# andabi/parallel-wavenet-vocoder

Measured on AMD Instinct MI355X. Metric: audio samples/sec, 4-flow IAF generation, higher is better.
Workload: dtype f32 via 3-term split-fp16 MFMA (fp32 accumulate, fp32 storage)

## Files before the change

parallel-wavenet-vocoder_amd/csrc/pwv_f16x3.h:

```cpp
#pragma once

#include "pwv_layer_common.h"

namespace pwv {

typedef float f32x2 __attribute__((ext_vector_type(2)));

template <int OFF, int N>
__device__ __forceinline__ void split8(const float (&x)[N], f16x8& hi, f16x8& lo) {
#pragma unroll
    for (int q = 0; q < 8; q += 2) {
        const f32x2 v = {x[OFF + q], x[OFF + q + 1]};
        const f16x2 h = __builtin_convertvector(v, f16x2);
        f32x2 r;
        asm("v_fma_mix_f32 %0, %1, -1.0, %2 op_sel:[0,0,0] op_sel_hi:[1,0,0]" : "=v"(r[0]) : "v"(h), "v"(v[0]));
        asm("v_fma_mix_f32 %0, %1, -1.0, %2 op_sel:[1,0,0] op_sel_hi:[1,0,0]" : "=v"(r[1]) : "v"(h), "v"(v[1]));
        const f16x2 l = __builtin_convertvector(r, f16x2);
        hi[q] = h[0];
        hi[q + 1] = h[1];
        lo[q] = l[0];
        lo[q + 1] = l[1];
    }
}

template <int NS, int NITTOT>
__device__ __forceinline__ f16x8 frag16(const f16x8* A, int comp, int it, int s, int lane) {
    return A[((comp * NITTOT + it) * NS + s) * 64 + lane];
}

template <int NS, int NIT, int IT0, int ITSTEP, int NITTOT, int NACC, typename BH, typename BL, typename EF, typename TF>
__device__ __forceinline__ void gemm16(const f16x8* A, int lane, f32x16 (&acc)[NACC], f16x8 (&ah)[4], f16x8 (&al)[4],
                                       BH&& bh, BL&& bl, EF&& extra, TF&& tail) {
#pragma unroll
    for (int s = 0; s < NS; ++s) {
        f16x8 nh[4] = {ah[0], ah[1], ah[2], ah[3]};
        f16x8 nl[4] = {al[0], al[1], al[2], al[3]};
        if (s + 1 < NS) {
#pragma unroll
            for (int i = 0; i < NIT; ++i) {
                nh[i] = frag16<NS, NITTOT>(A, 0, IT0 + i * ITSTEP, s + 1, lane);
                nl[i] = frag16<NS, NITTOT>(A, 1, IT0 + i * ITSTEP, s + 1, lane);
            }
        } else {
            tail(nh, nl);
        }
        __builtin_amdgcn_sched_barrier(0);
// ... 53 lines not shown
            ah[i] = nh[i];
            al[i] = nl[i];
        }
    }
}

template <int NS, int S, int NIT, int IT0, int ITSTEP, int NITTOT>
__device__ __forceinline__ void frags_at(const f16x8* A, int lane, f16x8 (&h)[4], f16x8 (&l)[4]) {
#pragma unroll
    for (int i = 0; i < NIT; ++i) {
        h[i] = frag16<NS, NITTOT>(A, 0, IT0 + i * ITSTEP, S, lane);
        l[i] = frag16<NS, NITTOT>(A, 1, IT0 + i * ITSTEP, S, lane);
    }
}

template <int NS, int NIT, int IT0, int ITSTEP, int NITTOT>
__device__ __forceinline__ void first_frags(const f16x8* A, int lane, f16x8 (&h)[4], f16x8 (&l)[4]) {
#pragma unroll
    for (int i = 0; i < NIT; ++i) {
        h[i] = frag16<NS, NITTOT>(A, 0, IT0 + i * ITSTEP, 0, lane);
        l[i] = frag16<NS, NITTOT>(A, 1, IT0 + i * ITSTEP, 0, lane);
    }
}

}
```

parallel-wavenet-vocoder_amd/csrc/pwv_head_f32.inc:

```
            PWV_HEAD_FENCE();
            f32x16 accs[4];
#pragma unroll
            for (int it = 0; it < 4; ++it)
#pragma unroll
                for (int q = 0; q < 4; ++q) {
                    const f32x4 v = *reinterpret_cast<const f32x4*>(hb + kHBS + h * 64 + it * 16 + q * 4);
#pragma unroll
                    for (int e = 0; e < 4; ++e) accs[it][q * 4 + e] = v[e];
                }
#pragma unroll
            for (int r = 0; r < 16; ++r) o[16 + r] = gate_act(acc[1][r], acc[3][r]);
            gemm_groups<8, 4, 0, 1>(lds, kHS, lane, accs, a, [&](int ks) -> float { return o[ks]; }, no_extra,
                                    [&](f32x4(&n)[4]) {
#pragma unroll
                                        for (int i = 0; i < 4; ++i) n[i] = frag(lds, kH1, i, 16, 0, lane);
                                    });
            PWV_HEAD_FENCE();
#pragma unroll
            for (int it = 0; it < 4; ++it)
#pragma unroll
                for (int q = 0; q < 4; ++q) {
                    const f32x4 v = *reinterpret_cast<const f32x4*>(hb + kHB1 + h * 64 + it * 16 + q * 4);
#pragma unroll
                    for (int e = 0; e < 4; ++e) acc1[it][q * 4 + e] = v[e];
                }
            gemm_groups<16, 4, 0, 1>(
                lds, kH1, lane, acc1, a, [&](int ks) -> float { return fmaxf(accs[ks >> 4][ks & 15], 0.f); }, no_extra,
                [](f32x4(&)[4]) {});
```

parallel-wavenet-vocoder_amd/csrc/pwv_layer_common.h:

```cpp
#pragma once

#include "pwv_common.h"

namespace pwv {

constexpr int kA1 = 0;
constexpr int kA1Size = 4 * 16 * 64 * 4;
constexpr int kA2 = kA1 + kA1Size;
constexpr int kA2Size = 2 * 8 * 64 * 4;
constexpr int kBD = kA2 + kA2Size;
constexpr int kBDSize = 64;
constexpr int kLayerBase = kBD + kBDSize;
constexpr int kASSize = 4 * 8 * 64 * 4;
constexpr int kBSSize = 128;
constexpr int kCondC = 80;
constexpr int kACSize = 4 * (kCondC / 8) * 64 * 4;

constexpr int layer_floats(bool skip, bool cond) {
    return kLayerBase + (skip ? kASSize + kBSSize : 0) + (cond ? kACSize : 0);
}

constexpr int kHAS = 0;
constexpr int kHBS = kHAS + kASSize;
constexpr int kHA1 = kHBS + kBSSize;
// ... 207 lines not shown
template <int NCH>
__device__ __forceinline__ void load_contig(const float* __restrict__ p, float (&dst)[4 * NCH]) {
#pragma unroll
    for (int g = 0; g < NCH; ++g) {
        const f32x4 v = *reinterpret_cast<const f32x4*>(p + 4 * g);
#pragma unroll
        for (int e = 0; e < 4; ++e) dst[4 * g + e] = v[e];
    }
}


__device__ __forceinline__ f32x4 frag(const float* lds, int base, int it, int ngroups, int g, int lane) {
    return *reinterpret_cast<const f32x4*>(&lds[base + ((it * ngroups + g) * 64 + lane) * 4]);
}

template <int NG, int NIT, int IT0, int ITSTEP, int NACC, typename BF, typename EF, typename TF>
__device__ __forceinline__ void gemm_groups(const float* lds, int base, int lane, f32x16 (&acc)[NACC], f32x4 (&a)[4],
                                            BF&& bval, EF&& extra, TF&& tail) {
#pragma unroll
    for (int g = 0; g < NG; ++g) {
        f32x4 n[4] = {a[0], a[1], a[2], a[3]};
        if (g + 1 < NG) {
#pragma unroll
            for (int i = 0; i < NIT; ++i) n[i] = frag(lds, base, IT0 + i * ITSTEP, NG, g + 1, lane);
        } else {
            tail(n);
        }
        __builtin_amdgcn_sched_barrier(0);
#pragma unroll
        for (int e = 0; e < 4; ++e) {
            const float b = bval(g * 4 + e);
#pragma unroll
// ... 28 lines not shown
```

parallel-wavenet-vocoder_amd/csrc/pwv_layer_f32_body.inc:

```
    static_assert(!FOLD || FIRST, "FOLD: layer 0 of a scalar-input net only");
    static_assert(!STREAM || (!SKIP && !COND && FOLD == FIRST && GATED == HEAD), "STREAM: folded layer 0, plain residual layer, last layer + head");
    static_assert(!HEAD || (GATED && !SKIP && !COND && !FIRST), "HEAD: plain last layer only");
    static_assert(!FIRST || !SKIP, "FIRST: no skip accumulation");
    constexpr int WAVES = 8;
    constexpr int kLds = HEAD ? kA1Size + kASSize + kHA1Size : layer_floats(SKIP, COND);
    constexpr int kCF = kLds + 4;
    constexpr int kHS = kA1Size;
    constexpr int kH1 = kA1Size + kASSize;
    __shared__ __attribute__((aligned(16))) float lds[kLds + (HEAD ? 0 : 4) + (FIRST ? 128 : 0)];

    const int tid = threadIdx.x;
    const int lane = tid & 63;
    const int wave = __builtin_amdgcn_readfirstlane(tid >> 6);
    const int h = lane >> 5;
    const int net = blockIdx.x % p.G;
    const int wg = blockIdx.x / p.G;
    const int nwg = gridDim.x / p.G;
    int* unit_counter = reinterpret_cast<int*>(&lds[HEAD ? 0 : kLds]);

    if constexpr (HEAD) {
        fill_lds_dma<kA1Size / 4, WAVES>(lds, p.packed[net] + kA1, wave, lane);
        fill_lds_dma<kASSize / 4, WAVES>(lds + kHS, p.packed_head[net] + kHAS, wave, lane);
        fill_lds_dma<kHA1Size / 4, WAVES>(lds + kH1, p.packed_head[net] + kHA1, wave, lane);
    } else {
// ... 151 lines not shown
                    n[1] = frag(lds, kA2, 1, 8, 0, lane);
                } else if constexpr (SKIP) {
#pragma unroll
                    for (int i = 0; i < 4; ++i) n[i] = frag(lds, kAS, i, 8, 0, lane);
                } else if constexpr (HEAD) {
#pragma unroll
                    for (int i = 0; i < 4; ++i) n[i] = frag(lds, kHS, i, 8, 0, lane);
                }
            });
        }

        const int ooff = units_off(cur.row, h, 64, u_begin);
        if constexpr (GATED && HEAD) {
            const float* hb = p.packed_head[net];
            f32x16 acc1[4];
#define PWV_HEAD_FENCE() do {} while (0)
#include "pwv_head_f32.inc"
#undef PWV_HEAD_FENCE
            const int Q = p.head_q;
            const int hq = h * Q;
#define PWV_HEAD_STORE(q, part) if (cur.valid && h == 0) p.head_out[net][(size_t)cur.row * Q + (q)] = (part)
#include "pwv_head_pp2.inc"
#undef PWV_HEAD_STORE
        } else if constexpr (GATED) {
            if constexpr (SKIP) load_skip_row<SKIP, COND>(p, net, lane, cur, skip_load);
#pragma unroll
            for (int r = 0; r < 16; ++r) o[16 + r] = gate_act(acc[1][r], acc[3][r]);
            if (cur.valid) {
#pragma unroll
                for (int g = 0; g < 8; ++g) {
// ... 79 lines not shown
```

parallel-wavenet-vocoder_amd/csrc/pwv_persist_fold0.inc:

```
    if (p.x_first && p.fold0[net]) {
        const float* Af = lds;
        const f16x8* A2 = reinterpret_cast<const f16x8*>(lds + kA1Size);
        (void)Af;
        (void)A2;
        const float* bias = lds + kBiasF + h * 32;
        const char* F0 = reinterpret_cast<const char*>(p.fold0[net]);
        const float* lastfrag = packed_n + kSlot + lane * 4;
        const int d = dil_of(0);
        const int dn = dil_next(0);
        typedef const __attribute__((address_space(3))) f32x4* lds_f4_t;
        const lds_f4_t cfb = (lds_f4_t)(lds + kCfF + 4 * h);
        f16x8 fh[4], fl[4];
        f32x4 ff[4];
#pragma unroll
        for (int it = 0; it < 4; ++it) {
            if constexpr (F32) {
                ff[it] = *reinterpret_cast<const f32x4*>(F0 + it * 1024 + lane * 16);
            } else {
                fh[it] = *reinterpret_cast<const f16x8*>(F0 + it * 1024 + lane * 16);
                fl[it] = *reinterpret_cast<const f16x8*>(F0 + (4 + it) * 1024 + lane * 16);
            }
        }
        const f32x4 lf32 = *reinterpret_cast<const f32x4*>(lastfrag);
        while (u >= 0 && j == 0) {
// ... 34 lines not shown
                int prow = 0;
                if (p.cond_hop > 0) prow = p_base(nn) + fast_div(t + p.cond_offset, p.hop_magic, p.hop_shift);
                const float* pr = proj_n + (size_t)prow * p.proj_row_stride + h * 64;
#pragma unroll
                for (int it = 0; it < 4; ++it)
#pragma unroll
                    for (int q = 0; q < 4; ++q) {
                        const f32x4 v = *reinterpret_cast<const f32x4*>(pr + it * 16 + q * 4);
#pragma unroll
                        for (int e = 0; e < 4; ++e) acc[it][q * 4 + e] = v[e];
                    }
            }
            int j2 = 0;
            const int u2 = next_task(0, u, j2);
            asm volatile("s_waitcnt vmcnt(0)" ::: "memory");
            publish();
            if (u2 >= 0 && !stat) claim_v = claim();
            if (p.range_flag && !(fabsf(x0) <= p.x_limit)) __hip_atomic_store(p.range_flag, 1, __ATOMIC_RELAXED, __HIP_MEMORY_SCOPE_SYSTEM);
            if constexpr (F32) {
                const float b0 = h ? xd0 : xd1, b1 = h ? x0 : x1v;
#pragma unroll
                for (int it = 0; it < 4; ++it) acc[it] = __builtin_amdgcn_mfma_f32_32x32x2f32(ff[it][0], b0, acc[it], 0, 0, 0);
#pragma unroll
                for (int it = 0; it < 4; ++it) acc[it] = __builtin_amdgcn_mfma_f32_32x32x2f32(ff[it][1], b1, acc[it], 0, 0, 0);
            } else {
                f16x8 b_h = {0, 0, 0, 0, 0, 0, 0, 0}, b_l = {0, 0, 0, 0, 0, 0, 0, 0};
                const float sc[4] = {xd1, xd0, x1v, x0};
#pragma unroll
                for (int q = 0; q < 4; ++q) {
                    const float v = h == 0 ? sc[q] : 0.f;
// ... 77 lines not shown
```

parallel-wavenet-vocoder_amd/csrc/pwv_persist_geometry.inc:

```
    constexpr bool SHORT = MODE == 2;
    __shared__ __attribute__((aligned(16))) float lds[kLdsFloats];
    const int tid = threadIdx.x;
    const int lane = tid & 63;
    const int wave = __builtin_amdgcn_readfirstlane(tid >> 6);
    const int h = lane >> 5;

    int net, w;
    if (p.xcd_map) {
        const int x = blockIdx.x & 7, s = blockIdx.x >> 3;
        net = s % p.G;
        w = x * (p.nwg >> 3) + s / p.G;
    } else {
        net = blockIdx.x % p.G;
        w = blockIdx.x / p.G;
    }
    const int rows = p.N * p.T;
    auto rows_of = [&](int unit, int& row, bool& valid, int& rc, int& nn, int& t) {
        if constexpr (VARLEN) unit_rows_varlen(p.unit_map, unit, lane, rows, row, valid, rc, nn, t);
        else unit_rows(unit, lane, rows, p.N, p.T, p.T_magic, p.T_shift, row, valid, rc, nn, t);
    };
    constexpr int kLaneStride = kMaxPLayers, kLaneHopMagic = kMaxPLayers + 1, kLaneHopShift = kMaxPLayers + 2, kLaneCondOffset = kMaxPLayers + 3,
                  kLaneCondFrames = kMaxPLayers + 4;
    static_assert(kMaxPLayers + 5 <= 64, "the dilations and the P row's scalars share one VGPR");
    int v_dil = p.dil[lane & (kMaxPLayers - 1)];
    if constexpr (!SHORT) {
        const int k = lane - kMaxPLayers;
        const int c = k == 0 ? p.proj_row_stride : (k == 1 ? (int)p.hop_magic : (k == 2 ? (int)p.hop_shift : (k == 3 ? p.cond_offset : p.cond_frames)));
        v_dil = k >= 0 ? c : v_dil;
    }
    auto dil_of = [&](int j) -> int { return __builtin_amdgcn_readlane(v_dil, j); };
    auto top_scalar = [&](int k) -> int { return __builtin_amdgcn_readlane(v_dil, k); };
    (void)top_scalar;
    auto p_base = [&](int nn) -> int {
        if constexpr (VARLEN) return nn;
        else if constexpr (SHORT) return nn * p.cond_frames;
        else return nn * top_scalar(kLaneCondFrames);
    };
    constexpr bool RAGGED = VARLEN && STREAM;
    auto unit_rec = [&](int unit, int& s0, int& r1) {
        typedef const __attribute__((address_space(4))) int* const_ints_t;
        const int last = (rows - 1) >> 5;
        const const_ints_t rec = (const_ints_t)(p.unit_map + (size_t)(unit < last ? unit : last) * kVarlenRec);
// ... 3 lines not shown
    auto session_end = [&](int s0, int r1, bool second) -> int {
        return second ? p.cu_rows[s0 + 2] : r1;
    };
    (void)unit_rec;
    (void)session_end;
    const int u_begin = w * p.per_wg;
    const int u_end = u_begin + p.per_wg < p.units ? u_begin + p.per_wg : p.units;
    const int n = u_end - u_begin;
    if (n <= 0) return;
    const int L = p.n_layers;
    constexpr bool stat = SHORT;
    constexpr bool loader_mode = SHORT;
#ifdef PWV_PTRACE
    int pt_nev = 0;
#endif

    typedef __attribute__((address_space(3))) int* lds_ints_t;
    const lds_ints_t ctl = (lds_ints_t)(lds + kCtlF);
    typedef __attribute__((address_space(3))) volatile unsigned char* lds_bytes_t;
    const lds_bytes_t lb = (lds_bytes_t)lds;
    int* prog_n = p.prog + (size_t)net * p.nwg * kProgStride;
    int* uprog_n = p.uprog + (size_t)net * p.units * kUnitStride;
    const float* const proj_n = p.proj[net];
    const float* const packed_n = p.packed[net];
    auto dil_next = [&](int j) -> int { return j + 1 < L ? dil_of(j + 1) : (p.tail_q > 0 ? p.tail_dil : dil_of(j)); };

    for (int k = tid; k < (kLdsFloats - kCtlF); k += 512) ctl[k] = 0;
    __syncthreads();
    if (tid == 0) {
        lb[kSeenLB] = w > 0 ? 0 : 255;
        lb[kSeenRB] = w < p.last_wg ? 0 : 255;
        lb[kWreadyB] = 0;
        lb[kWreadyB + 1] = 1;
        lb[kTrueB] = 255;
    }
    auto fill_slot = [&](int slot, int layer, int first, int step) {
        const float* src = packed_n + (size_t)layer * p.packed_stride + lane * 4;
        float* dst = lds + slot * kSlot;
        if constexpr (!SHORT) {
            const __amdgpu_buffer_rsrc_t prs = __builtin_amdgcn_make_buffer_rsrc((void*)(packed_n + (size_t)layer * p.packed_stride), 0, (kSlotFull + 64) * 4, 0x00020000);
#pragma clang loop unroll(disable)
            for (int c = first; c < kSlot / 256; c += step)
                __builtin_amdgcn_raw_ptr_buffer_load_lds(prs, (lptr_t)(dst + c * 256), 16, lane * 16, c * 1024, 0, 0);
            if (first == 0 && lane < 16) __builtin_amdgcn_raw_ptr_buffer_load_lds(prs, (lptr_t)(lds + kBiasF + slot * 64), 16, lane * 16, kSlotFull * 4, 0, 0);
            return;
        }
#pragma clang loop unroll(disable)
        for (int c = first; c < kSlot / 256; c += step)
            __builtin_amdgcn_global_load_lds((gptr_t)(src + c * 256), (lptr_t)(dst + c * 256), 16, 0, 0);
        if (first == 0 && lane < 16)
            __builtin_amdgcn_global_load_lds((gptr_t)(src + kSlotFull), (lptr_t)(lds + kBiasF + slot * 64), 16, 0, 0);
    };
    if (p.x_first && tid < 128) lds[kCfF + tid] = p.cfilt[net][tid];
    fill_slot(0, 0, wave, 8);
    if (L > 1) fill_slot(1, 1, wave, 8);
    __syncthreads();
    if (wave >= 4) __builtin_amdgcn_s_setprio(1);

    const __amdgpu_buffer_rsrc_t ring_rs = [&]() {
        const unsigned long long a = (unsigned long long)p.ring[net];
        const unsigned long long span = (unsigned long long)p.ring_stride * 8ull + (unsigned long long)p.units * 8192ull;
        const unsigned lo = __builtin_amdgcn_readfirstlane((unsigned)a), hi2 = __builtin_amdgcn_readfirstlane((unsigned)(a >> 32));
        return __builtin_amdgcn_make_buffer_rsrc((void*)(((unsigned long long)hi2 << 32) | lo), 0, __builtin_amdgcn_readfirstlane((unsigned)span), 0x00020000);
    }();
    const __amdgpu_buffer_rsrc_t proj_rs = [&]() {
        const unsigned long long a = (unsigned long long)proj_n;
        const unsigned lo = __builtin_amdgcn_readfirstlane((unsigned)a), hi2 = __builtin_amdgcn_readfirstlane((unsigned)(a >> 32));
        return __builtin_amdgcn_make_buffer_rsrc((void*)(((unsigned long long)hi2 << 32) | lo), 0, 0xFFFFFFFFu, 0x00020000);
    }();
    (void)proj_rs;
    auto proj_rs_at = [&](long long floats) -> __amdgpu_buffer_rsrc_t {
// ... 153 lines not shown
```

parallel-wavenet-vocoder_amd/csrc/pwv_persist_loader.inc:

```
    if (loader_mode && wave == 7) {
        __builtin_amdgcn_s_setprio(0);
        bool gone = false;
        for (int jj = 0; jj < L && !gone; ++jj) {
            const long long t0 = __builtin_amdgcn_s_memrealtime();
            for (int k = 0;; ++k) {
                if (__builtin_amdgcn_readfirstlane(*(__attribute__((address_space(3))) volatile int*)&ctl[8 + jj]) >= n) break;
                if (__builtin_amdgcn_readfirstlane(*(__attribute__((address_space(3))) volatile int*)&ctl[1])) { gone = true; break; }
                if ((k & 63) == 63 && (__builtin_amdgcn_readfirstlane(__hip_atomic_load(p.abort, __ATOMIC_RELAXED, __HIP_MEMORY_SCOPE_AGENT)) ||
                                       __builtin_amdgcn_s_memrealtime() - t0 > kWaitTicks)) {
                    __hip_atomic_store(p.status, 7, __ATOMIC_RELAXED, __HIP_MEMORY_SCOPE_SYSTEM);
                    __hip_atomic_store(p.abort, 1, __ATOMIC_RELAXED, __HIP_MEMORY_SCOPE_AGENT);
                    *(__attribute__((address_space(3))) volatile int*)&ctl[1] = 1;
                    gone = true;
                    break;
                }
                __builtin_amdgcn_s_sleep(2);
            }
            if (gone) break;
            if (lane == 0) __hip_atomic_store(prog_n + (size_t)w * kProgStride, jj + 1, __ATOMIC_RELAXED, __HIP_MEMORY_SCOPE_AGENT);
            PT_EV(7, jj, -1);
            if (jj + 2 < L) {
                fill_slot(jj & 1, jj + 2, 0, 1);
                asm volatile("s_waitcnt vmcnt(0)" ::: "memory");
                lb[kWreadyB + (jj & 1)] = (unsigned char)(jj + 2);
            }
        }
    }
```

parallel-wavenet-vocoder_amd/csrc/pwv_persist_plan.h:

```cpp
#pragma once

#include <cstddef>

#include "pwv_hip.h"

#ifndef PWV_CHECK_ARG
#define PWV_CHECK_ARG(cond, ...)          \
    do {                                  \
        if (!(cond)) return PWV_EINVAL;   \
    } while (0)
#endif

namespace pwv {

constexpr int kLeftN = 32;
constexpr int kUnitModeMaxPerWg = 7;
constexpr int kUnitStride = 32;
constexpr int kMaxPLayers = 32;
constexpr int kProgStride = 32;
constexpr int kMaxReachWgs = 60;
constexpr int kMaxUnitsWg = 832;
constexpr int kPlanMaxQ = 4;

struct PersistPlan { int units, nwg, per_wg, last_wg, reach_wgs, xcd_map, tail_reach_wgs, unit_mode; };
// ... 28 lines not shown
    pl.unit_mode = 0;
    if (reach <= kLeftN && pl.nwg > 1 && pl.per_wg <= kUnitModeMaxPerWg) {
        pl.unit_mode = 2;
        PWV_CHECK_ARG(pl.reach_wgs <= 32, "persistent stack: unit mode polls at most 32 right neighbours (reach %d workgroups)", pl.reach_wgs);
    }
    pl.tail_reach_wgs = 0;
    if (tail_q > 0) {
        PWV_CHECK_ARG(tail_q <= kPlanMaxQ && tail_dil >= 1, "persistent stack: tail_q 1..%d, tail_dilation >= 1", kPlanMaxQ);
        PWV_CHECK_ARG(rows * tail_q * 4 < (1ll << 32), "persistent stack: tail_out beyond the 4 GB reach of a buffer descriptor");
        pl.tail_reach_wgs = ((tail_dil + 31) / 32 + pl.per_wg - 1) / pl.per_wg;
        PWV_CHECK_ARG(pl.tail_reach_wgs <= kMaxReachWgs, "persistent stack: tail dilation %d reaches over %d workgroups (max %d)", tail_dil, pl.tail_reach_wgs, kMaxReachWgs);
    }
    return PWV_OK;
}

struct PersistLayout { size_t prog_bytes, pair_off, uprog_off, total; };

inline size_t align256(size_t v) { return (v + 255) & ~(size_t)255; }

inline PersistLayout persist_layout(int G, const PersistPlan& pl) {
    PersistLayout l;
    l.prog_bytes = (size_t)G * pl.nwg * kProgStride * 4;
    l.pair_off = align256(l.prog_bytes + 256);
    l.uprog_off = l.pair_off + align256((size_t)pl.nwg * 4);
    l.total = l.uprog_off + (pl.unit_mode ? align256((size_t)G * pl.units * kUnitStride * 4) : 0);
    return l;
}

}
```

parallel-wavenet-vocoder_amd/csrc/pwv_persist_protocol.inc:

```

    int vpack = 0;
    auto layer_vectors = [&](int j) {
        const int d = dil_of(j), d2 = dil_of(j >= 2 ? j - 2 : 0);
        const int off = lane == 1 ? -((d + 31) >> 5) : (lane == 2 ? -(d >> 5) : (lane == 4 ? (d2 >> 5) : (lane == 5 ? ((d2 + 31) >> 5) : 0)));
        const int raw = j >= 1 ? j : 0, wts = j >= 2 ? j : 0, war = j >= 2 ? j - 1 : 0;
        const int need = lane < 3 ? raw : (lane == 3 ? wts : (lane < 6 ? war : 0));
        vpack = (need << 16) | (off & 0xffff);
    };
    auto dep_addr = [&](int j, int u) -> int {
        const int v = u + (int)(short)vpack;
        int a = kDoneB - u_begin + v;
        a = (v < u_begin && !SHORT) ? kSeenLB : a;
        a = v >= u_end ? kSeenRB : a;
        a = (v < 0 || v >= p.units) ? kTrueB : a;
        a = lane == 3 ? kWreadyB + (j & 1) : a;
        return lane >= 6 ? kTrueB : a;
    };
    auto eval = [&](int addr) -> unsigned { return (unsigned)__ballot((int)lb[addr] < (vpack >> 16)); };
    auto wave_min = [&](int v) -> int {
#pragma unroll
        for (int o = 32; o >= 1; o >>= 1) { const int t = __shfl_xor(v, o); v = t < v ? t : v; }
        return v;
    };
    auto poll_side = [&](int side, int need) {
// ... 20 lines not shown
            v = __hip_atomic_load(uprog_n + (size_t)(u_begin - kLeftN + addr - kLeftB) * kUnitStride, __ATOMIC_RELAXED, __HIP_MEMORY_SCOPE_AGENT);
        } else if (lo >= 32 && lo - 32 < cnt_r) {
            v = __hip_atomic_load(prog_n + (size_t)(w + 1 + lo - 32) * kProgStride, __ATOMIC_RELAXED, __HIP_MEMORY_SCOPE_AGENT);
        }
        v = v > 255 ? 255 : v;
        if (left) lb[addr] = (unsigned char)v;
        if (cnt_r > 0) {
            const bool r = lo >= 32;
            if (__ballot(r && v < jw + 1) == 0) lb[kSeenRB] = (unsigned char)(jw + 1);
            else if (__ballot(r && v < jw) == 0 && (int)lb[kSeenRB] < jw) lb[kSeenRB] = (unsigned char)jw;
        }
    };

    int prev_addr = -1, prev_j = 0;
    int dma_pending = -1;
    int left_upto = 0;
    bool dead = false;
    auto publish = [&]() {
        if (prev_addr >= 0) {
            lb[prev_addr] = (unsigned char)(prev_j + 1);
            if (SHORT && lane == 0) __hip_atomic_store(uprog_n + (size_t)(prev_addr - kDoneB + u_begin) * kUnitStride, prev_j + 1, __ATOMIC_RELAXED, __HIP_MEMORY_SCOPE_AGENT);
            prev_addr = -1;
        }
        if (dma_pending >= 0) { lb[kWreadyB + (dma_pending & 1)] = (unsigned char)dma_pending; dma_pending = -1; }
    };
    auto flush_owed = [&]() {
        asm volatile("s_waitcnt vmcnt(0)" ::: "memory");
        publish();
    };
    auto leave_layers = [&](int upto) {
        for (; left_upto < upto; ++left_upto) {
            const int jj = left_upto;
            int old = 0;
            if (lane == 0) old = __hip_atomic_fetch_add(&ctl[8 + jj], 1, __ATOMIC_RELAXED, __HIP_MEMORY_SCOPE_WORKGROUP);
            old = __builtin_amdgcn_readfirstlane(old);
            if (old == 7 && !loader_mode) {
                if (lane == 0) __hip_atomic_store(prog_n + (size_t)w * kProgStride, jj + 1, __ATOMIC_RELAXED, __HIP_MEMORY_SCOPE_AGENT);
                PT_EV(7, jj, -1);
                if (jj + 2 < L) {
                    if (dma_pending >= 0) flush_owed();
                    fill_slot(jj & 1, jj + 2, 0, 1);
                    dma_pending = jj + 2;
                }
            }
        }
    };
    auto wait_deps = [&](int j, int u, unsigned mask, int lv, int code) {
        if (!SHORT || prev_addr >= 0 || dma_pending >= 0) {
            flush_owed();
            PT_EV(mask == kWarMask ? 13 : 3, j, u);
        }
        leave_layers(j);
        if (dma_pending >= 0) flush_owed();
        if (lv != j) layer_vectors(j);
        const int addr = dep_addr(j, u);
        bool ok = false;
        const long long t0 = __builtin_amdgcn_s_memrealtime();
// ... 56 lines not shown
```

parallel-wavenet-vocoder_amd/csrc/pwv_persist_tail.inc:

```
    bool tail_done = false;
    {
        if (p.tail_q > 0) {
            tail_done = true;
            PT_EV(8, L, -1);
            __syncthreads();
            const int wg_dead = __builtin_amdgcn_readfirstlane(*(__attribute__((address_space(3))) volatile int*)&ctl[1]);
            __syncthreads();
            bool tail_ok = !wg_dead;
            if (tail_ok) {
                constexpr int kHS = kA1Size, kH1 = kA1Size + kASSize;
                fill_lds_dma<kA1Size / 4, 8>(lds, p.tail_layer[net] + kA1, wave, lane);
                fill_lds_dma<kASSize / 4, 8>(lds + kHS, p.tail_head[net] + kHAS, wave, lane);
                fill_lds_dma<kHA1Size / 4, 8>(lds + kH1, p.tail_head[net] + kHA1, wave, lane);
                const int td = p.tail_dil;
                if (w > 0 && wave < ((td + 31) >> 5)) {
                    const int w0 = w - p.tail_reach_wgs > 0 ? w - p.tail_reach_wgs : 0;
                    const int cnt = w - w0;
                    const long long t0 = __builtin_amdgcn_s_memrealtime();
                    for (int k = 0;; ++k) {
                        int v = 1 << 20;
                        if (lane < cnt) v = __hip_atomic_load(prog_n + (size_t)(w0 + lane) * kProgStride, __ATOMIC_RELAXED, __HIP_MEMORY_SCOPE_AGENT);
                        if (__ballot(v < L) == 0) break;
                        if ((k & 63) == 63 && (__builtin_amdgcn_readfirstlane(__hip_atomic_load(p.abort, __ATOMIC_RELAXED, __HIP_MEMORY_SCOPE_AGENT)) ||
                                               __builtin_amdgcn_s_memrealtime() - t0 > kWaitTicks)) {
                            __hip_atomic_store(p.status, 6, __ATOMIC_RELAXED, __HIP_MEMORY_SCOPE_SYSTEM);
                            __hip_atomic_store(p.abort, 1, __ATOMIC_RELAXED, __HIP_MEMORY_SCOPE_AGENT);
                            tail_ok = false;
                            break;
                        }
                        __builtin_amdgcn_s_sleep(4);
                    }
                }
                asm volatile("s_waitcnt vmcnt(0)" ::: "memory");
                __syncthreads();
                PT_EV(9, L, -1);
                const f16x8* A1 = reinterpret_cast<const f16x8*>(lds);
                const f16x8* HS = reinterpret_cast<const f16x8*>(lds + kHS);
                const f16x8* H1 = reinterpret_cast<const f16x8*>(lds + kH1);
                (void)A1; (void)HS; (void)H1;
                const float* hb = p.tail_head[net];
                const int Q = p.tail_q;
                const int so = in_soff(L);
                const __amdgpu_buffer_rsrc_t out_rs = [&]() {
                    const unsigned long long a = (unsigned long long)p.tail_out[net];
                    const unsigned lo = __builtin_amdgcn_readfirstlane((unsigned)a), hi2 = __builtin_amdgcn_readfirstlane((unsigned)(a >> 32));
                    return __builtin_amdgcn_make_buffer_rsrc((void*)(((unsigned long long)hi2 << 32) | lo), 0,
                                                             __builtin_amdgcn_readfirstlane((unsigned)rows * (unsigned)Q * 4u), 0x00020000);
                }();
                auto load_tail = [&](int unit, float (&xb)[32], float (&xc)[32]) {
                    int row, rc, nn, t;
                    bool valid;
                    rows_of(unit, row, valid, rc, nn, t);
                    const bool has_prev = t >= td;
                    const int oc = toff(rc), ob = toff(has_prev ? rc - td : rc);
// ... 24 lines not shown
                    hist_store(L, td, nn, t, unit, rc, valid, txc);
                    f32x16 acc[4];
                    {
                        int prow = 0;
                        if (p.cond_hop > 0) prow = p_base(nn) + fast_div(t + p.cond_offset, p.hop_magic, p.hop_shift);
                        const float* pr = proj_n + (size_t)prow * p.proj_row_stride + L * 128 + h * 64;
#pragma unroll
                        for (int it = 0; it < 4; ++it)
#pragma unroll
                            for (int q = 0; q < 4; ++q) {
                                const f32x4 v = *reinterpret_cast<const f32x4*>(pr + it * 16 + q * 4);
#pragma unroll
                                for (int e = 0; e < 4; ++e) acc[it][q * 4 + e] = v[e];
                            }
                    }
                    f32x16 acc1[4];
                    if constexpr (F32) {
                        auto bx = [&](int ks) -> float { return ks < 32 ? txb[ks] : txc[ks - 32]; };
                        float o[32];
                        f32x4 a[4];
                        a[0] = frag(lds, 0, 0, 16, 0, lane);
                        a[1] = frag(lds, 0, 2, 16, 0, lane);
                        gemm_groups<16, 2, 0, 2>(lds, 0, lane, acc, a, bx, no_extra, [&](f32x4(&nf)[4]) {
                            nf[0] = frag(lds, 0, 1, 16, 0, lane);
                            nf[1] = frag(lds, 0, 3, 16, 0, lane);
                        });
                        gemm_groups<16, 2, 1, 2>(
                            lds, 0, lane, acc, a, bx,
                            [&](int g) {
                                o[g] = gate_act(acc[0][g], acc[2][g]);
                                asm volatile("" : "+v"(o[g]));
                            },
                            [&](f32x4(&nf)[4]) {
#pragma unroll
                                for (int i = 0; i < 4; ++i) nf[i] = frag(lds, kHS, i, 8, 0, lane);
                            });
#define PWV_HEAD_FENCE() asm volatile("" ::: "memory")
#include "pwv_head_f32.inc"
#undef PWV_HEAD_FENCE
                    } else {
                        f16x8 bh[8], bl[8];
                        float xc[32];
#pragma unroll
                        for (int i = 0; i < 32; ++i) xc[i] = txc[i];
                        split8<0>(xc, bh[4], bl[4]);
                        split8<8>(xc, bh[5], bl[5]);
                        split8<16>(xc, bh[6], bl[6]);
                        split8<24>(xc, bh[7], bl[7]);
                        auto bxh = [&](int s) -> f16x8 { return bh[s ^ 4]; };
                        auto bxl = [&](int s) -> f16x8 { return bl[s ^ 4]; };
// ... 79 lines not shown
```

parallel-wavenet-vocoder_amd/csrc/pwv_persist_tasks.inc:

```
    if (u >= 0) {
        flush_owed();
        leave_layers(j);
        layer_vectors(j);
        if constexpr (SHORT) {
            load_xc(j, u, rxc);
        } else {
            const unsigned bad = eval(dep_addr(j, u));
            if (bad & kRawMask) wait_deps(j, u, kRawMask, j, 4);
            war_ok = (bad & kWarMask) == 0;
            if (!dead) load_x(j, u, rxb, rxc);
        }
    }
    int lv_j = j;

    while (u >= 0 && !dead) {
        PT_MARK();
        PT_BEGIN();
        int row, rc, nn, t;
        bool valid;
        rows_of_top(u, row, valid, rc, nn, t);
        if constexpr (SHORT) {
            flush_owed();
            PT_EV(3, j, u);
            leave_layers(j);
// ... 196 lines not shown
```

parallel-wavenet-vocoder_amd/csrc/pwv_stack_persist.hip:

```cpp
#include "pwv_f16x3.h"
#include "pwv_persist_plan.h"

#include <cstddef>
#include <cstdlib>
#include <cstring>

namespace pwv {

constexpr int kStoreAuxLocal = 0;

constexpr int kSlotFull = kA1Size + kA2Size;
constexpr int kSlot = kSlotFull - 256;
constexpr int kBiasF = 2 * kSlot;
constexpr int kCtlF = kBiasF + 128;
constexpr int kCtlInts = 40;
constexpr int kLdsFloats = 40960;
constexpr int kCfF = kCtlF + kCtlInts;
constexpr int kLeftB = (kCfF + 128) * 4;
constexpr int kDoneB = kLeftB + kLeftN;
constexpr int kMaxUnitsWgLds = kLdsFloats * 4 - kDoneB;
static_assert(kMaxUnitsWg == kMaxUnitsWgLds && kPlanMaxQ == kMaxQ, "pwv_persist_plan.h restates the kernel's limits");
static_assert(kUnitModeMaxPerWg <= 7, "the short-input instantiation keeps wave 7 as its loader");
static_assert(kLeftN <= 32, "unit mode: the right neighbours are polled by lanes 32..63 alone");
constexpr int kFlagB = (kCtlF + 2) * 4;
constexpr int kSeenLB = kFlagB, kSeenRB = kFlagB + 1, kWreadyB = kFlagB + 2, kTrueB = kFlagB + 4;
constexpr long long kWaitTicks = 2000000;

struct PersistParams {
    float* ring[PWV_MAX_NETS];
    long long ring_stride;
    const float* packed[PWV_MAX_NETS];
    const float* proj[PWV_MAX_NETS];
    int* prog;
    int* uprog;
    int unit_mode;
    int* abort;
// ... 17 lines not shown
    const float* tail_layer[PWV_MAX_NETS];
    const float* tail_head[PWV_MAX_NETS];
    float* tail_out[PWV_MAX_NETS];
    int tail_q, tail_dil, tail_reach_wgs;
    const float* affine_x;
    float* affine_out;
    int* pair;
    const int* unit_map;
    const float* hist_rd;
    float* hist_wr;
    const int* slot_tab;
    long long hist_block_stride;
    long long hist_scalar_off;
    long long hist_off[PWV_MAX_NETS][kMaxPLayers + 1];
    const int* cu_rows;
};

#ifdef PWV_PTRACE
#define PT_DECL long long pt_acc[18] = {0, 0, 0, 0, 0, 0, 0, 0, 0, 0, 0, 0, 0, 0, 0, 0, 0, 0}; long long pt_t = 0, pt_p = 0; (void)pt_t; (void)pt_p;
#define PT_BEGIN() pt_t = __builtin_amdgcn_s_memtime()
#define PT_END(k) pt_acc[k] += __builtin_amdgcn_s_memtime() - pt_t
#define PT_ADD(k, v) pt_acc[k] += (v)
#define PT_LAP(k) do { __builtin_amdgcn_sched_barrier(0); const long long pt_n = __builtin_amdgcn_s_memtime(); pt_acc[k] += pt_n - pt_t; pt_t = pt_n; __builtin_amdgcn_sched_barrier(0); } while (0)
#define PT_MARK() do { __builtin_amdgcn_sched_barrier(0); pt_p = __builtin_amdgcn_s_memtime(); __builtin_amdgcn_sched_barrier(0); } while (0)
#define PT_PHASE(k) do { __builtin_amdgcn_sched_barrier(0); const long long pt_n = __builtin_amdgcn_s_memtime(); pt_acc[k] += pt_n - pt_p; pt_p = pt_n; __builtin_amdgcn_sched_barrier(0); } while (0)
#define PT_EV(code, jj, uu) do { if (p.trace_ev && pt_nev < 64) { if (lane == 0) { long long* e_ = p.trace_ev + (((size_t)blockIdx.x * 8 + wave) * 64 + pt_nev) * 4; \
    e_[0] = __builtin_amdgcn_s_memrealtime(); e_[1] = (code); e_[2] = (jj); e_[3] = (long long)(uu); } ++pt_nev; } } while (0)
#else
#define PT_DECL
#define PT_BEGIN() do {} while (0)
#define PT_END(k) do {} while (0)
#define PT_ADD(k, v) do {} while (0)
#define PT_LAP(k) do {} while (0)
#define PT_MARK() do {} while (0)
#define PT_PHASE(k) do {} while (0)
#define PT_EV(code, jj, uu) do {} while (0)
#endif

constexpr unsigned kRawMask = 0xFu, kWarMask = 0x30u;

template <typename FR, typename BH, typename BL, typename EF>
// ... 331 lines not shown
        const int n_hist = a->n_layers + (a->tail_q > 0 ? 1 : 0);
        for (int g = 0; g < a->G; ++g)
            for (int j = a->x_first ? 1 : 0; j < n_hist; ++j) {
                const size_t off = a->hist_row_off[g][j];
                const size_t hist_rows = ((size_t)(j < a->n_layers ? a->dilations[j] : a->tail_dilation) + 31) / 32 * 32;
                PWV_CHECK_ARG(off % 4 == 0 && off + hist_rows * 64 <= sa.block_stride,
                              "pwv_wavenet_stack_persist_f32: hist_row_off[%d][%d] + round32(dilation) rows leave the history block", g, j);
                p.hist_off[g][j] = (long long)off;
            }
    }
    p.trace = nullptr;
#ifdef PWV_PTRACE
    { const char* e = getenv("PWV_PTRACE_PTR"); if (e) p.trace = (long long*)strtoull(e, nullptr, 0); }
    p.trace_ev = nullptr;
    { const char* e = getenv("PWV_PTRACE_EV_PTR"); if (e) p.trace_ev = (long long*)strtoull(e, nullptr, 0); }
#endif
    hipStream_t s = (hipStream_t)stream;
    const size_t n16 = r.lay.total / 16;
    if (!a->workspace_clean)
        hipLaunchKernelGGL(persist_zero_kernel, dim3((unsigned)((n16 + 255) / 256)), dim3(256), 0, s, (int4*)a->workspace, n16);
    const dim3 grid(a->G * pl.nwg), block(512);
    const persist_kernel_t kernel = (ragged ? kRagged : streaming ? kStreaming : varlen ? kPacked : kUniform)[a->precision == PWV_PREC_F32][pl.unit_mode == 2];
    hipLaunchKernelGGL(kernel, grid, block, 0, s, p);
    hipError_t e = hipGetLastError();
    if (e != hipSuccess) return set_error(PWV_EHIP, "persistent stack kernel launch failed: %s", hipGetErrorString(e));
    return PWV_OK;
}

int pwv_varlen_unit_map(const int* cu_rows, const int* cu_frames, int n_utt, int units, int* out, pwv_stream_t stream) {
    PWV_CHECK_ARG(cu_rows && out, "pwv_varlen_unit_map: NULL argument");
// ... 10 lines not shown
```

Measured before the change: 58.19 million.

## Prefetch tail A1 matrix into free weight slot and defer slot-1 startup wait

The persistent kernel's loader now DMA-prefetches the tail layer's first matrix into the free double-buffer slot during the last layer. The tail head's skip matrix is split across two LDS regions via a parity-dependent map, so the tail no longer reloads A1 synchronously. The start barrier also waits only for slot 0's loads, and slot 1's readiness is signalled later by a per-wave counter. This moves weight-load latency off the tail and startup critical path, at the cost of more complex LDS placement and synchronisation logic.

```diff
diff --git a/parallel-wavenet-vocoder_amd/csrc/pwv_f16x3.h b/parallel-wavenet-vocoder_amd/csrc/pwv_f16x3.h
--- a/parallel-wavenet-vocoder_amd/csrc/pwv_f16x3.h
+++ b/parallel-wavenet-vocoder_amd/csrc/pwv_f16x3.h
@@ -23,13 +23,19 @@
     }
 }
 
-template <int NS, int NITTOT>
-__device__ __forceinline__ f16x8 frag16(const f16x8* A, int comp, int it, int s, int lane) {
+template <int SPLIT>
+struct SplitLdsF16 {
+    const f16x8* lo;
+    const f16x8* hi;
+    __device__ __forceinline__ f16x8 operator[](int i) const { return i < SPLIT * 64 ? lo[i] : hi[i]; }
+};
+template <int NS, int NITTOT, typename AP>
+__device__ __forceinline__ f16x8 frag16(AP A, int comp, int it, int s, int lane) {
     return A[((comp * NITTOT + it) * NS + s) * 64 + lane];
 }
 
-template <int NS, int NIT, int IT0, int ITSTEP, int NITTOT, int NACC, typename BH, typename BL, typename EF, typename TF>
-__device__ __forceinline__ void gemm16(const f16x8* A, int lane, f32x16 (&acc)[NACC], f16x8 (&ah)[4], f16x8 (&al)[4],
+template <int NS, int NIT, int IT0, int ITSTEP, int NITTOT, int NACC, typename BH, typename BL, typename EF, typename TF, typename AP>
+__device__ __forceinline__ void gemm16(AP A, int lane, f32x16 (&acc)[NACC], f16x8 (&ah)[4], f16x8 (&al)[4],
                                        BH&& bh, BL&& bl, EF&& extra, TF&& tail) {
 #pragma unroll
     for (int s = 0; s < NS; ++s) {
@@ -113,8 +119,8 @@
     }
 }
 
-template <int NS, int NIT, int IT0, int ITSTEP, int NITTOT>
-__device__ __forceinline__ void first_frags(const f16x8* A, int lane, f16x8 (&h)[4], f16x8 (&l)[4]) {
+template <int NS, int NIT, int IT0, int ITSTEP, int NITTOT, typename AP>
+__device__ __forceinline__ void first_frags(AP A, int lane, f16x8 (&h)[4], f16x8 (&l)[4]) {
 #pragma unroll
     for (int i = 0; i < NIT; ++i) {
         h[i] = frag16<NS, NITTOT>(A, 0, IT0 + i * ITSTEP, 0, lane);
diff --git a/parallel-wavenet-vocoder_amd/csrc/pwv_head_f32.inc b/parallel-wavenet-vocoder_amd/csrc/pwv_head_f32.inc
--- a/parallel-wavenet-vocoder_amd/csrc/pwv_head_f32.inc
+++ b/parallel-wavenet-vocoder_amd/csrc/pwv_head_f32.inc
@@ -10,10 +10,10 @@
                 }
 #pragma unroll
             for (int r = 0; r < 16; ++r) o[16 + r] = gate_act(acc[1][r], acc[3][r]);
-            gemm_groups<8, 4, 0, 1>(lds, kHS, lane, accs, a, [&](int ks) -> float { return o[ks]; }, no_extra,
+            gemm_groups<8, 4, 0, 1>(ldsS, kHS, lane, accs, a, [&](int ks) -> float { return o[ks]; }, no_extra,
                                     [&](f32x4(&n)[4]) {
 #pragma unroll
-                                        for (int i = 0; i < 4; ++i) n[i] = frag(lds, kH1, i, 16, 0, lane);
+                                        for (int i = 0; i < 4; ++i) n[i] = frag(lds1, kH1, i, 16, 0, lane);
                                     });
             PWV_HEAD_FENCE();
 #pragma unroll
@@ -25,5 +25,5 @@
                     for (int e = 0; e < 4; ++e) acc1[it][q * 4 + e] = v[e];
                 }
             gemm_groups<16, 4, 0, 1>(
-                lds, kH1, lane, acc1, a, [&](int ks) -> float { return fmaxf(accs[ks >> 4][ks & 15], 0.f); }, no_extra,
+                lds1, kH1, lane, acc1, a, [&](int ks) -> float { return fmaxf(accs[ks >> 4][ks & 15], 0.f); }, no_extra,
                 [](f32x4(&)[4]) {});
diff --git a/parallel-wavenet-vocoder_amd/csrc/pwv_layer_common.h b/parallel-wavenet-vocoder_amd/csrc/pwv_layer_common.h
--- a/parallel-wavenet-vocoder_amd/csrc/pwv_layer_common.h
+++ b/parallel-wavenet-vocoder_amd/csrc/pwv_layer_common.h
@@ -245,8 +245,19 @@
     return *reinterpret_cast<const f32x4*>(&lds[base + ((it * ngroups + g) * 64 + lane) * 4]);
 }
 
-template <int NG, int NIT, int IT0, int ITSTEP, int NACC, typename BF, typename EF, typename TF>
-__device__ __forceinline__ void gemm_groups(const float* lds, int base, int lane, f32x16 (&acc)[NACC], f32x4 (&a)[4],
+template <int SPLIT>
+struct SplitLdsF32 {
+    const float* lo;
+    const float* hi;
+    __device__ __forceinline__ const float& operator[](int i) const { return i < SPLIT * 256 ? lo[i] : hi[i]; }
+};
+template <int SPLIT>
+__device__ __forceinline__ f32x4 frag(const SplitLdsF32<SPLIT>& lds, int base, int it, int ngroups, int g, int lane) {
+    return *reinterpret_cast<const f32x4*>(&lds[base + ((it * ngroups + g) * 64 + lane) * 4]);
+}
+
+template <int NG, int NIT, int IT0, int ITSTEP, int NACC, typename BF, typename EF, typename TF, typename LP>
+__device__ __forceinline__ void gemm_groups(LP lds, int base, int lane, f32x16 (&acc)[NACC], f32x4 (&a)[4],
                                             BF&& bval, EF&& extra, TF&& tail) {
 #pragma unroll
     for (int g = 0; g < NG; ++g) {
diff --git a/parallel-wavenet-vocoder_amd/csrc/pwv_layer_f32_body.inc b/parallel-wavenet-vocoder_amd/csrc/pwv_layer_f32_body.inc
--- a/parallel-wavenet-vocoder_amd/csrc/pwv_layer_f32_body.inc
+++ b/parallel-wavenet-vocoder_amd/csrc/pwv_layer_f32_body.inc
@@ -189,6 +189,8 @@
         if constexpr (GATED && HEAD) {
             const float* hb = p.packed_head[net];
             f32x16 acc1[4];
+            const float* const ldsS = lds;
+            const float* const lds1 = lds;
 #define PWV_HEAD_FENCE() do {} while (0)
 #include "pwv_head_f32.inc"
 #undef PWV_HEAD_FENCE
diff --git a/parallel-wavenet-vocoder_amd/csrc/pwv_persist_fold0.inc b/parallel-wavenet-vocoder_amd/csrc/pwv_persist_fold0.inc
--- a/parallel-wavenet-vocoder_amd/csrc/pwv_persist_fold0.inc
+++ b/parallel-wavenet-vocoder_amd/csrc/pwv_persist_fold0.inc
@@ -1,3 +1,7 @@
+    if (u < 0 && start_owed) {
+        asm volatile("s_waitcnt vmcnt(0)" ::: "memory");
+        start_landed();
+    }
     if (p.x_first && p.fold0[net]) {
         const float* Af = lds;
         const f16x8* A2 = reinterpret_cast<const f16x8*>(lds + kA1Size);
@@ -72,6 +76,7 @@
             int j2 = 0;
             const int u2 = next_task(0, u, j2);
             asm volatile("s_waitcnt vmcnt(0)" ::: "memory");
+            if (start_owed) start_landed();
             publish();
             if (u2 >= 0 && !stat) claim_v = claim();
             if (p.range_flag && !(fabsf(x0) <= p.x_limit)) __hip_atomic_store(p.range_flag, 1, __ATOMIC_RELAXED, __HIP_MEMORY_SCOPE_SYSTEM);
diff --git a/parallel-wavenet-vocoder_amd/csrc/pwv_persist_geometry.inc b/parallel-wavenet-vocoder_amd/csrc/pwv_persist_geometry.inc
--- a/parallel-wavenet-vocoder_amd/csrc/pwv_persist_geometry.inc
+++ b/parallel-wavenet-vocoder_amd/csrc/pwv_persist_geometry.inc
@@ -20,12 +20,14 @@
         else unit_rows(unit, lane, rows, p.N, p.T, p.T_magic, p.T_shift, row, valid, rc, nn, t);
     };
     constexpr int kLaneStride = kMaxPLayers, kLaneHopMagic = kMaxPLayers + 1, kLaneHopShift = kMaxPLayers + 2, kLaneCondOffset = kMaxPLayers + 3,
-                  kLaneCondFrames = kMaxPLayers + 4;
-    static_assert(kMaxPLayers + 5 <= 64, "the dilations and the P row's scalars share one VGPR");
+                  kLaneCondFrames = kMaxPLayers + 4, kLaneTailLo = kMaxPLayers + 5, kLaneTailHi = kMaxPLayers + 6;
+    static_assert(kMaxPLayers + 7 <= 64, "the dilations, the P row's scalars and the tail's first matrix share one VGPR");
     int v_dil = p.dil[lane & (kMaxPLayers - 1)];
     if constexpr (!SHORT) {
         const int k = lane - kMaxPLayers;
-        const int c = k == 0 ? p.proj_row_stride : (k == 1 ? (int)p.hop_magic : (k == 2 ? (int)p.hop_shift : (k == 3 ? p.cond_offset : p.cond_frames)));
+        const unsigned long long ta = p.tail_q > 0 ? (unsigned long long)p.tail_layer[net] : 0ull;
+        const int c = k == 0 ? p.proj_row_stride : (k == 1 ? (int)p.hop_magic : (k == 2 ? (int)p.hop_shift : (k == 3 ? p.cond_offset : (k == 4 ? p.cond_frames :
+                      (k == 5 ? (int)(unsigned)ta : (int)(unsigned)(ta >> 32))))));
         v_dil = k >= 0 ? c : v_dil;
     }
     auto dil_of = [&](int j) -> int { return __builtin_amdgcn_readlane(v_dil, j); };
@@ -59,6 +61,7 @@
 #ifdef PWV_PTRACE
     int pt_nev = 0;
 #endif
+    PT_EV(19, 0, -1);
 
     typedef __attribute__((address_space(3))) int* lds_ints_t;
     const lds_ints_t ctl = (lds_ints_t)(lds + kCtlF);
@@ -76,7 +79,7 @@
         lb[kSeenLB] = w > 0 ? 0 : 255;
         lb[kSeenRB] = w < p.last_wg ? 0 : 255;
         lb[kWreadyB] = 0;
-        lb[kWreadyB + 1] = 1;
+        lb[kWreadyB + 1] = SHORT ? 1 : 0;
         lb[kTrueB] = 255;
     }
     auto fill_slot = [&](int slot, int layer, int first, int step) {
@@ -96,10 +99,31 @@
         if (first == 0 && lane < 16)
             __builtin_amdgcn_global_load_lds((gptr_t)(src + kSlotFull), (lptr_t)(lds + kBiasF + slot * 64), 16, 0, 0);
     };
+    auto fill_tail_a1 = [&](int slot) {
+        float* dst = lds + slot * kSlot;
+        unsigned long long src = (unsigned long long)(unsigned)top_scalar(kLaneTailLo) | ((unsigned long long)(unsigned)top_scalar(kLaneTailHi) << 32);
+        asm volatile("" : "+s"(src));
+        const __amdgpu_buffer_rsrc_t prs = __builtin_amdgcn_make_buffer_rsrc((void*)src, 0, kA1Size * 4, 0x00020000);
+#pragma clang loop unroll(disable)
+        for (int c = 0; c < kA1Size / 256; ++c)
+            __builtin_amdgcn_raw_ptr_buffer_load_lds(prs, (lptr_t)(dst + c * 256), 16, lane * 16, c * 1024, 0, 0);
+    };
+    (void)fill_tail_a1;
     if (p.x_first && tid < 128) lds[kCfF + tid] = p.cfilt[net][tid];
+    static_assert(kSlot / 256 == 79, "the shares of slot 1 below: chunks wave, wave + 8, ... < 79");
     fill_slot(0, 0, wave, 8);
-    if (L > 1) fill_slot(1, 1, wave, 8);
-    __syncthreads();
+    fill_slot(1, 1, wave, 8);
+    if constexpr (SHORT) {
+        __syncthreads();
+    } else {
+        asm volatile("s_waitcnt lgkmcnt(0)" ::: "memory");
+        if (wave == 0) asm volatile("s_waitcnt vmcnt(11)" ::: "memory");
+        else if (wave == 7) asm volatile("s_waitcnt vmcnt(9)" ::: "memory");
+        else asm volatile("s_waitcnt vmcnt(10)" ::: "memory");
+        __builtin_amdgcn_s_barrier();
+        asm volatile("" ::: "memory");
+    }
+    PT_EV(21, 0, -1);
     if (wave >= 4) __builtin_amdgcn_s_setprio(1);
 
     const __amdgpu_buffer_rsrc_t ring_rs = [&]() {
diff --git a/parallel-wavenet-vocoder_amd/csrc/pwv_persist_loader.inc b/parallel-wavenet-vocoder_amd/csrc/pwv_persist_loader.inc
--- a/parallel-wavenet-vocoder_amd/csrc/pwv_persist_loader.inc
+++ b/parallel-wavenet-vocoder_amd/csrc/pwv_persist_loader.inc
@@ -23,6 +23,7 @@
                 fill_slot(jj & 1, jj + 2, 0, 1);
                 asm volatile("s_waitcnt vmcnt(0)" ::: "memory");
                 lb[kWreadyB + (jj & 1)] = (unsigned char)(jj + 2);
+                PT_EV(20, jj + 2, -1);
             }
         }
     }
diff --git a/parallel-wavenet-vocoder_amd/csrc/pwv_persist_plan.h b/parallel-wavenet-vocoder_amd/csrc/pwv_persist_plan.h
--- a/parallel-wavenet-vocoder_amd/csrc/pwv_persist_plan.h
+++ b/parallel-wavenet-vocoder_amd/csrc/pwv_persist_plan.h
@@ -66,6 +66,22 @@
     return PWV_OK;
 }
 
+constexpr int kPlanLdsFloats = 40960;
+constexpr int kPlanSlotFloats = 20224;
+constexpr int kPlanTailA1Floats = 16384, kPlanTailSkipFloats = 8192, kPlanTailPost1Floats = 16384;
+constexpr int kFragFloats = 256;
+constexpr int kTailSkipSplit = (kPlanSlotFloats - kPlanTailPost1Floats) / kFragFloats;
+static_assert(kPlanTailA1Floats + kPlanTailSkipFloats + kPlanTailPost1Floats == kPlanLdsFloats, "the head's three matrices are the whole LDS");
+static_assert(kPlanSlotFloats + kPlanTailA1Floats + kPlanTailSkipFloats - kTailSkipSplit * kFragFloats == kPlanLdsFloats, "the skip matrix's upper piece ends with the LDS");
+
+struct TailMap { int a1, post1, hs_lo, hs_hi; };
+
+constexpr TailMap persist_tail_map(int n_layers) {
+    return (n_layers & 1) == 0
+               ? TailMap{0, kPlanTailA1Floats + kPlanTailSkipFloats, kPlanTailA1Floats, kPlanTailA1Floats}
+               : TailMap{kPlanSlotFloats, 0, kPlanTailPost1Floats, kPlanSlotFloats + kPlanTailA1Floats - kTailSkipSplit * kFragFloats};
+}
+
 struct PersistLayout { size_t prog_bytes, pair_off, uprog_off, total; };
 
 inline size_t align256(size_t v) { return (v + 255) & ~(size_t)255; }
diff --git a/parallel-wavenet-vocoder_amd/csrc/pwv_persist_protocol.inc b/parallel-wavenet-vocoder_amd/csrc/pwv_persist_protocol.inc
--- a/parallel-wavenet-vocoder_amd/csrc/pwv_persist_protocol.inc
+++ b/parallel-wavenet-vocoder_amd/csrc/pwv_persist_protocol.inc
@@ -3,7 +3,7 @@
     auto layer_vectors = [&](int j) {
         const int d = dil_of(j), d2 = dil_of(j >= 2 ? j - 2 : 0);
         const int off = lane == 1 ? -((d + 31) >> 5) : (lane == 2 ? -(d >> 5) : (lane == 4 ? (d2 >> 5) : (lane == 5 ? ((d2 + 31) >> 5) : 0)));
-        const int raw = j >= 1 ? j : 0, wts = j >= 2 ? j : 0, war = j >= 2 ? j - 1 : 0;
+        const int raw = j >= 1 ? j : 0, wts = j >= (SHORT ? 2 : 1) ? j : 0, war = j >= 2 ? j - 1 : 0;
         const int need = lane < 3 ? raw : (lane == 3 ? wts : (lane < 6 ? war : 0));
         vpack = (need << 16) | (off & 0xffff);
     };
@@ -58,15 +58,25 @@
 
     int prev_addr = -1, prev_j = 0;
     int dma_pending = -1;
+    bool start_owed = !SHORT;
     int left_upto = 0;
     bool dead = false;
+    auto start_landed = [&]() {
+        start_owed = false;
+        int old = 0;
+        if (lane == 0) old = __hip_atomic_fetch_add(&ctl[5], 1, __ATOMIC_RELAXED, __HIP_MEMORY_SCOPE_WORKGROUP);
+        if (__builtin_amdgcn_readfirstlane(old) == 7) {
+            lb[kWreadyB + 1] = 1;
+            PT_EV(20, 1, -1);
+        }
+    };
     auto publish = [&]() {
         if (prev_addr >= 0) {
             lb[prev_addr] = (unsigned char)(prev_j + 1);
             if (SHORT && lane == 0) __hip_atomic_store(uprog_n + (size_t)(prev_addr - kDoneB + u_begin) * kUnitStride, prev_j + 1, __ATOMIC_RELAXED, __HIP_MEMORY_SCOPE_AGENT);
             prev_addr = -1;
         }
-        if (dma_pending >= 0) { lb[kWreadyB + (dma_pending & 1)] = (unsigned char)dma_pending; dma_pending = -1; }
+        if (dma_pending >= 0) { lb[kWreadyB + (dma_pending & 1)] = (unsigned char)dma_pending; PT_EV(20, dma_pending, -1); dma_pending = -1; }
     };
     auto flush_owed = [&]() {
         asm volatile("s_waitcnt vmcnt(0)" ::: "memory");
@@ -85,6 +95,10 @@
                     if (dma_pending >= 0) flush_owed();
                     fill_slot(jj & 1, jj + 2, 0, 1);
                     dma_pending = jj + 2;
+                } else if (jj + 2 == L && (top_scalar(kLaneTailLo) | top_scalar(kLaneTailHi)) != 0) {
+                    if (dma_pending >= 0) flush_owed();
+                    fill_tail_a1(jj & 1);
+                    dma_pending = L;
                 }
             }
         }
diff --git a/parallel-wavenet-vocoder_amd/csrc/pwv_persist_tail.inc b/parallel-wavenet-vocoder_amd/csrc/pwv_persist_tail.inc
--- a/parallel-wavenet-vocoder_amd/csrc/pwv_persist_tail.inc
+++ b/parallel-wavenet-vocoder_amd/csrc/pwv_persist_tail.inc
@@ -8,10 +8,11 @@
             __syncthreads();
             bool tail_ok = !wg_dead;
             if (tail_ok) {
-                constexpr int kHS = kA1Size, kH1 = kA1Size + kASSize;
-                fill_lds_dma<kA1Size / 4, 8>(lds, p.tail_layer[net] + kA1, wave, lane);
-                fill_lds_dma<kASSize / 4, 8>(lds + kHS, p.tail_head[net] + kHAS, wave, lane);
-                fill_lds_dma<kHA1Size / 4, 8>(lds + kH1, p.tail_head[net] + kHA1, wave, lane);
+                const TailMap tm = persist_tail_map(SHORT ? 0 : L);
+                if constexpr (SHORT) fill_lds_dma<kA1Size / 4, 8>(lds + tm.a1, p.tail_layer[net] + kA1, wave, lane);
+                fill_lds_dma<kTailSkipSplit * 64, 8>(lds + tm.hs_lo, p.tail_head[net] + kHAS, wave, lane);
+                fill_lds_dma<kASSize / 4 - kTailSkipSplit * 64, 8>(lds + tm.hs_hi + kTailSkipSplit * kFragFloats, p.tail_head[net] + kHAS + kTailSkipSplit * kFragFloats, wave, lane);
+                fill_lds_dma<kHA1Size / 4, 8>(lds + tm.post1, p.tail_head[net] + kHA1, wave, lane);
                 const int td = p.tail_dil;
                 if (w > 0 && wave < ((td + 31) >> 5)) {
                     const int w0 = w - p.tail_reach_wgs > 0 ? w - p.tail_reach_wgs : 0;
@@ -34,10 +35,14 @@
                 asm volatile("s_waitcnt vmcnt(0)" ::: "memory");
                 __syncthreads();
                 PT_EV(9, L, -1);
-                const f16x8* A1 = reinterpret_cast<const f16x8*>(lds);
-                const f16x8* HS = reinterpret_cast<const f16x8*>(lds + kHS);
-                const f16x8* H1 = reinterpret_cast<const f16x8*>(lds + kH1);
-                (void)A1; (void)HS; (void)H1;
+                const f16x8* A1 = reinterpret_cast<const f16x8*>(lds + tm.a1);
+                const SplitLdsF16<kTailSkipSplit> HS = {reinterpret_cast<const f16x8*>(lds + tm.hs_lo), reinterpret_cast<const f16x8*>(lds + tm.hs_hi)};
+                const f16x8* H1 = reinterpret_cast<const f16x8*>(lds + tm.post1);
+                const float* const ldsA = lds + tm.a1;
+                const SplitLdsF32<kTailSkipSplit> ldsS = {lds + tm.hs_lo, lds + tm.hs_hi};
+                const float* const lds1 = lds + tm.post1;
+                constexpr int kHS = 0, kH1 = 0;
+                (void)A1; (void)HS; (void)H1; (void)ldsA; (void)ldsS; (void)lds1; (void)kHS; (void)kH1;
                 const float* hb = p.tail_head[net];
                 const int Q = p.tail_q;
                 const int so = in_soff(L);
@@ -92,26 +97,27 @@
                                 for (int e = 0; e < 4; ++e) acc[it][q * 4 + e] = v[e];
                             }
                     }
+                    if (unit == u_begin + wave) PT_EV(22, L, unit);
                     f32x16 acc1[4];
                     if constexpr (F32) {
                         auto bx = [&](int ks) -> float { return ks < 32 ? txb[ks] : txc[ks - 32]; };
                         float o[32];
                         f32x4 a[4];
-                        a[0] = frag(lds, 0, 0, 16, 0, lane);
-                        a[1] = frag(lds, 0, 2, 16, 0, lane);
-                        gemm_groups<16, 2, 0, 2>(lds, 0, lane, acc, a, bx, no_extra, [&](f32x4(&nf)[4]) {
-                            nf[0] = frag(lds, 0, 1, 16, 0, lane);
-                            nf[1] = frag(lds, 0, 3, 16, 0, lane);
+                        a[0] = frag(ldsA, 0, 0, 16, 0, lane);
+                        a[1] = frag(ldsA, 0, 2, 16, 0, lane);
+                        gemm_groups<16, 2, 0, 2>(ldsA, 0, lane, acc, a, bx, no_extra, [&](f32x4(&nf)[4]) {
+                            nf[0] = frag(ldsA, 0, 1, 16, 0, lane);
+                            nf[1] = frag(ldsA, 0, 3, 16, 0, lane);
                         });
                         gemm_groups<16, 2, 1, 2>(
-                            lds, 0, lane, acc, a, bx,
+                            ldsA, 0, lane, acc, a, bx,
                             [&](int g) {
                                 o[g] = gate_act(acc[0][g], acc[2][g]);
                                 asm volatile("" : "+v"(o[g]));
                             },
                             [&](f32x4(&nf)[4]) {
 #pragma unroll
-                                for (int i = 0; i < 4; ++i) nf[i] = frag(lds, kHS, i, 8, 0, lane);
+                                for (int i = 0; i < 4; ++i) nf[i] = frag(ldsS, kHS, i, 8, 0, lane);
                             });
 #define PWV_HEAD_FENCE() asm volatile("" ::: "memory")
 #include "pwv_head_f32.inc"
diff --git a/parallel-wavenet-vocoder_amd/csrc/pwv_persist_tasks.inc b/parallel-wavenet-vocoder_amd/csrc/pwv_persist_tasks.inc
--- a/parallel-wavenet-vocoder_amd/csrc/pwv_persist_tasks.inc
+++ b/parallel-wavenet-vocoder_amd/csrc/pwv_persist_tasks.inc
@@ -1,5 +1,6 @@
     if (u >= 0) {
         flush_owed();
+        if (start_owed) start_landed();
         leave_layers(j);
         layer_vectors(j);
         if constexpr (SHORT) {
diff --git a/parallel-wavenet-vocoder_amd/csrc/pwv_stack_persist.hip b/parallel-wavenet-vocoder_amd/csrc/pwv_stack_persist.hip
--- a/parallel-wavenet-vocoder_amd/csrc/pwv_stack_persist.hip
+++ b/parallel-wavenet-vocoder_amd/csrc/pwv_stack_persist.hip
@@ -20,6 +20,8 @@
 constexpr int kDoneB = kLeftB + kLeftN;
 constexpr int kMaxUnitsWgLds = kLdsFloats * 4 - kDoneB;
 static_assert(kMaxUnitsWg == kMaxUnitsWgLds && kPlanMaxQ == kMaxQ, "pwv_persist_plan.h restates the kernel's limits");
+static_assert(kPlanSlotFloats == kSlot && kPlanLdsFloats == kLdsFloats && kPlanTailA1Floats == kA1Size && kPlanTailSkipFloats == kASSize &&
+              kPlanTailPost1Floats == kHA1Size && kA1 == 0, "pwv_persist_plan.h restates the sizes its tail map is made of");
 static_assert(kUnitModeMaxPerWg <= 7, "the short-input instantiation keeps wave 7 as its loader");
 static_assert(kLeftN <= 32, "unit mode: the right neighbours are polled by lanes 32..63 alone");
 constexpr int kFlagB = (kCtlF + 2) * 4;
@@ -67,6 +69,9 @@
     long long hist_scalar_off;
     long long hist_off[PWV_MAX_NETS][kMaxPLayers + 1];
     const int* cu_rows;
+#ifdef PWV_PTRACE
+    unsigned long long trace_codes;
+#endif
 };
 
 #ifdef PWV_PTRACE
@@ -77,7 +82,7 @@
 #define PT_LAP(k) do { __builtin_amdgcn_sched_barrier(0); const long long pt_n = __builtin_amdgcn_s_memtime(); pt_acc[k] += pt_n - pt_t; pt_t = pt_n; __builtin_amdgcn_sched_barrier(0); } while (0)
 #define PT_MARK() do { __builtin_amdgcn_sched_barrier(0); pt_p = __builtin_amdgcn_s_memtime(); __builtin_amdgcn_sched_barrier(0); } while (0)
 #define PT_PHASE(k) do { __builtin_amdgcn_sched_barrier(0); const long long pt_n = __builtin_amdgcn_s_memtime(); pt_acc[k] += pt_n - pt_p; pt_p = pt_n; __builtin_amdgcn_sched_barrier(0); } while (0)
-#define PT_EV(code, jj, uu) do { if (p.trace_ev && pt_nev < 64) { if (lane == 0) { long long* e_ = p.trace_ev + (((size_t)blockIdx.x * 8 + wave) * 64 + pt_nev) * 4; \
+#define PT_EV(code, jj, uu) do { if (p.trace_ev && pt_nev < 64 && ((p.trace_codes >> ((code) & 63)) & 1)) { if (lane == 0) { long long* e_ = p.trace_ev + (((size_t)blockIdx.x * 8 + wave) * 64 + pt_nev) * 4; \
     e_[0] = __builtin_amdgcn_s_memrealtime(); e_[1] = (code); e_[2] = (jj); e_[3] = (long long)(uu); } ++pt_nev; } } while (0)
 #else
 #define PT_DECL
@@ -439,6 +444,8 @@
     { const char* e = getenv("PWV_PTRACE_PTR"); if (e) p.trace = (long long*)strtoull(e, nullptr, 0); }
     p.trace_ev = nullptr;
     { const char* e = getenv("PWV_PTRACE_EV_PTR"); if (e) p.trace_ev = (long long*)strtoull(e, nullptr, 0); }
+    p.trace_codes = ~0ull;
+    { const char* e = getenv("PWV_PTRACE_EV_CODES"); if (e) p.trace_codes = strtoull(e, nullptr, 0); }
 #endif
     hipStream_t s = (hipStream_t)stream;
     const size_t n16 = r.lay.total / 16;
```

Result: no change. 58.28 million, median of 2 (+0.2%).
